# Tongdongq/darwin-gpu

Hardware: AMD Instinct MI355X
Metric: GACT GCUPS (DP cells/s) on ~10 kb PacBio-shape reads (higher is better)
Workload: dtype int16x2 (packed); 1 GPU; ecoli10x_self_overlap; tile_size=320, tile_overlap=120, scoring=+1/-1/-1/-1, reads=4642, bases=48503677, candidates=65766, tiles=2185214, parallelism=candidates dealt round-robin over 1 GPU(s), slots_in_flight=4, passes_in_this_process=127, arch=gfx950:sramecc+:xnack-

## Files before the change

darwin-gpu_amd/csrc/gact_coop.hpp:

```cpp
#pragma once

#include "gact_lin.hpp"

namespace gact {

constexpr int kCoopBanks = 2;
constexpr int kCoopJobs = (kBlockThreads / 64) * 8 * kCoopBanks;
static_assert(kCoopJobs == 64, "a walking wave serves every job of its block, one per lane");
constexpr int kCoopCacheStride = 36;

struct CoopJob {
    uint32_t ws_off;
    int R, Q;
    int k0;
    int v0;
    int band_lim;
    uint32_t where;
    int pad_;
};
struct CoopDone { int ref_steps, query_steps, dv, redo; };

template <class L> constexpr size_t coop_bank_words() { return (size_t)L::G::kMaxFlush * L::kWalkQuads * kWsRow * 4; }
template <class L> __host__ constexpr size_t coop_ws_words(int blocks) { return (size_t)blocks * (kBlockThreads / 64) * kCoopBanks * coop_bank_words<L>(); }

template <class L>
__device__ __forceinline__ void coop_walk_batch(const KParams &kp, const uint32_t *__restrict__ ws_all, const CoopJob *jobs, uint32_t *jstate,
                                                CoopDone *done, const uint32_t *stage_all, uint32_t *cache_all)
{
    constexpr int CW = L::kWalkCols, QN = L::kWalkQuads, ROW = kWsRow;
    constexpr int kSeg = StageGeom<L::kSlotsPerLane, L::kLanes>::kSeg;
    constexpr uint32_t kMagic = (65536u + CW - 1) / CW;
    constexpr uint32_t kM = 3u, kI = 2u, kD = 1u;
    typedef __attribute__((address_space(3))) const uint8_t LdsByte;
    typedef __attribute__((address_space(3))) const uint32_t LdsWord;
    const int lane = threadIdx.x & 63;
    uint32_t *scratch = cache_all + lane * kCoopCacheStride;
    LdsByte *cache = (LdsByte *)scratch;
    LdsWord *stage = (LdsWord *)stage_all;
    const int early = kp.early;
    int v_gap, v_mism, v_match;
    asm volatile("s_nop 1\n\tv_mov_b32 %0, %1" : "=v"(v_gap) : "s"(__builtin_amdgcn_readfirstlane(kp.ext)));
    asm volatile("s_nop 1\n\tv_mov_b32 %0, %1" : "=v"(v_mism) : "s"(__builtin_amdgcn_readfirstlane(kp.mismatch)));
    asm volatile("s_nop 1\n\tv_mov_b32 %0, %1" : "=v"(v_match) : "s"(__builtin_amdgcn_readfirstlane(kp.match)));

    const uint32_t st0 = __hip_atomic_load(&jstate[lane], __ATOMIC_RELAXED, __HIP_MEMORY_SCOPE_WORKGROUP);
    bool active = false;
    if ((st0 & 3u) == 1u) active = atomicCAS(&jstate[lane], st0, st0 + 1u) == st0;
    __builtin_amdgcn_fence(__ATOMIC_ACQUIRE, "workgroup");
    if (!__any(active)) return;
    int p0 = 0, kA = 0, nlim_i = 0, nlim_j = 0, nis = 0, njs = 0, v = 0, v0 = 0, band_lim = -1;
    uint32_t ws_off = 0;
    int rpos0 = 0, qpos0 = 0, dir = 0, seg = 0;
    int l = 0, c = 0, k = 0;
    bool go = false, redo = false;
    if (active) {
        const CoopJob jb = jobs[lane];
        const int R = jb.R, Q = jb.Q;
        ws_off = jb.ws_off; v0 = jb.v0; band_lim = jb.band_lim;
        int l0, c0, k0;
        L::walk_start(R, Q, 0, l0, c0, k0);
        k0 = jb.k0;
        p0 = l0 * CW + c0; kA = k0 - l0;
        nlim_i = -imin(early, R); nlim_j = -imin(early, Q);
        const bool rev = (jb.where >> 16) & 1u;
        seg = (int)(jb.where >> 17);
        dir = rev ? -1 : 1;
        rpos0 = (int)(jb.where & 0xffu) + (rev ? 0 : R - 1);
        qpos0 = (int)((jb.where >> 8) & 0xffu) + (rev ? 0 : Q - 1);
        v = v0;
        l = l0; c = c0; k = k0;
        go = (R >= 1) & (Q >= 1) & (early > 0) & (v != 0);
    }
    uint32_t cur = 0, rcode = 0, qcode = 0;
    TbRegion<CW> rg;
    rg.l0 = 0; rg.fbase[0] = rg.fbase[1] = rg.fbase[2] = 0; rg.qbase0 = 0;
    int off0 = 0, off1 = 0;
    auto fetch = [&](int fl, int fc, int fk) {
        const int off = fl == rg.l0 ? off0 : off1;
        const uint32_t row = ((uint32_t)fk >> 3 << 5) + (uint32_t)off;
        const uint32_t w = *(LdsWord *)(cache + (((uint32_t)fc >> 1 << 2) + row));
        return __builtin_amdgcn_ubfe(w, (((uint32_t)fc & 1u) << 4) + 14u - (((uint32_t)fk & 7u) << 1), 2u);
    };
    auto bases = [&]() {
        const int rp = rpos0 + dir * nis, qp = qpos0 + dir * njs;
        const uint32_t rw = stage[seg + (rp >> 4)], qw = stage[seg + kSeg + (qp >> 4)];
        rcode = __builtin_amdgcn_ubfe(rw, ((uint32_t)rp & 15u) << 1, 2u);
        qcode = __builtin_amdgcn_ubfe(qw, ((uint32_t)qp & 15u) << 1, 2u);
    };
#ifdef GACT_STAMPS
    unsigned long long n_trips = 0, n_lane_trips = 0;
#endif
    while (__any(go)) {
        if (go) {
            tb_refill_oct<CW, QN, ROW>(ws_all, ws_off, scratch, l, c, k, rg);
            off0 = 4 * (-8 * rg.fbase[0] - 4 * rg.qbase0);
            off1 = 4 * (16 - 8 * rg.fbase[1] - 4 * (QN - 2));
            cur = fetch(l, c, k);
            bases();
        }
#pragma unroll 1
        for (int m = 0; m < 8; m++) {
            if (!__any(go)) break;
#ifdef GACT_STAMPS
            n_trips++; n_lane_trips += (unsigned long long)__builtin_popcountll(__ballot(go));
#endif
            if (go) {
                const bool diag = cur == kM;
                const int sub = rcode == qcode ? v_match : v_mism;
                v -= diag ? sub : v_gap;
                nis -= cur != kD;
                njs -= cur != kI;
                const int p = imax(p0 + njs, 0);
                l = (int)(__umul24((uint32_t)p, kMagic) >> 16);
                c = p + __mul24(l, -CW);
                k = imax(kA + l + nis, 0);
                if (m == 7) {
                    redo = redo | ((band_lim >= 0) & ((unsigned)(nis - njs + band_lim) > (unsigned)(2 * band_lim)));
                } else {
                    cur = fetch(l, c, k);
                    bases();
                }
                go = !((diag && v == 0) || nis <= nlim_i || njs <= nlim_j || redo);
            }
        }
    }
    if (active) {
        done[lane].ref_steps = -nis; done[lane].query_steps = -njs; done[lane].dv = v0 - v; done[lane].redo = redo ? 1 : 0;
        __builtin_amdgcn_fence(__ATOMIC_RELEASE, "workgroup");
        __hip_atomic_store(&jstate[lane], st0 + 2u, __ATOMIC_RELAXED, __HIP_MEMORY_SCOPE_WORKGROUP);
    }
#ifdef GACT_STAMPS
    {
        const unsigned long long n_jobs = (unsigned long long)__builtin_popcountll(__ballot(active));
        if (lane == 0) { atomicAdd(&g_coop_counts[0], 1ull); atomicAdd(&g_coop_counts[1], n_trips); atomicAdd(&g_coop_counts[2], n_lane_trips);
                         atomicAdd(&g_coop_counts[3], n_jobs); }
    }
#endif
}

template <class L, bool TWO_SETS = false>
__global__ __launch_bounds__(kBlockThreads, 3) void extend_coop_kernel(
    KParams kp, P16Consts kc, SeqSetDev refs, SeqSetDev qfwd, SeqSetDev qrc,
    int same_file, gact_overlap *__restrict__ out, ChainQueues cq,
    uint32_t *__restrict__ ws_all)
{
    using G = typename L::G;
    constexpr int LANES = L::kLanes;
    static_assert(LANES == kGroup && L::kWalkFmt == 3 && L::kEndAligned, "the split linear-gap layout");
    constexpr int kGroupsOfWave = 64 / LANES;
    constexpr int kGroupsPerBlock = (kBlockThreads / 64) * kGroupsOfWave;
    constexpr int kStageWords = StageGeom<L::kSlotsPerLane, LANES>::kWords;
    constexpr int kSeg = StageGeom<L::kSlotsPerLane, LANES>::kSeg;
    static_assert(((kGroupsPerBlock * kCoopBanks * kStageWords) >> 15) == 0, "stage index fits CoopJob::where");
    constexpr int kRefBytes = (G::kRefBytes + 15) & ~15;
    __shared__ __attribute__((aligned(16))) uint8_t lds[kGroupsPerBlock * kRefBytes];
    __shared__ ChainState chain_lds[kGroupsPerBlock][kCoopBanks][kSlots];
    __shared__ __attribute__((aligned(16))) uint32_t stage_lds[kGroupsPerBlock][kCoopBanks][kStageWords];
    __shared__ __attribute__((aligned(16))) CoopJob jobs[kCoopJobs];
    __shared__ CoopDone done[kCoopJobs];
    __shared__ uint32_t jstate[kCoopJobs];
    __shared__ __attribute__((aligned(16))) uint32_t cache_lds[kCoopJobs * kCoopCacheStride];
    __shared__ int bank_lds[kGroupsPerBlock][kCoopBanks][6];
    __shared__ uint32_t walk_lock;

    uint32_t *const lin_lut = LinLutLds<L::kLutWords>::get();
    for (int n = threadIdx.x; n < kCoopJobs; n += kBlockThreads) jstate[n] = 0;
    if (threadIdx.x == 0) walk_lock = 0;
    lin_lut_fill_for_pass<L>(lin_lut, kc, (int)threadIdx.x);
    __syncthreads();

    const int wave_in_block = threadIdx.x >> 6;
    WaveCtx w;
    {
        const int lane = threadIdx.x & 63;
        w.gl = lane & (LANES - 1);
        w.g = lane / LANES;
        w.slot = (blockIdx.x * (kBlockThreads / 64) + wave_in_block) * kGroupsOfWave + w.g;
        w.n_slots = gridDim.x * (kBlockThreads / 64) * kGroupsOfWave;
    }
    const int group_in_block = wave_in_block * kGroupsOfWave + w.g;
    uint8_t *ref8 = lds + group_in_block * kRefBytes;
    uint8_t *q8 = ref8;
    const uint16_t *ref16_lane = reinterpret_cast<const uint16_t *>(ref8) + (L::kRow0 - 1 - w.gl);
    uint32_t *ws_wave = ws_all + (size_t)(blockIdx.x * (kBlockThreads / 64) + wave_in_block) * (kCoopBanks * coop_bank_words<L>());
    const int job_base = (group_in_block * kSlots + (w.gl & 1)) * kCoopBanks;

    for (int b = 0; b < kCoopBanks; b++)
        if (w.gl < kSlots) { chain_lds[group_in_block][b][w.gl].phase = 2; chain_lds[group_in_block][b][w.gl].cand = -1; }
    if (w.gl == 0) {
        int *bt = &bank_lds[group_in_block][0][0];
        for (int n = 0; n < kCoopBanks * 6; n++) bt[n] = 0;
    }
    wave_sync();
    bool exhausted = false;
    int my_bucket = 0;
    int bucket_first = 0;
    if (cq.leave_longest > 0) {
        int acc = 0;
        while (bucket_first < kBuckets && (acc += cq.bucket_count[bucket_first]) <= cq.leave_longest) bucket_first++;
        if (bucket_first >= kBuckets) bucket_first = 0;
    }
    bool second_set = false;
    constexpr bool one_set = !TWO_SETS;
    int idle_polls = 0;
    int rank_turn = 0, rank_cached = 0;
    int bank = 0;
    __builtin_amdgcn_s_setprio(3);
#ifdef GACT_STAMPS
    unsigned long long stamp_acc[8] = {0, 0, 0, 0, 0, 0, 0, 0};
    const unsigned long long tl_start = __builtin_amdgcn_s_memrealtime();
    const unsigned long long tl_cyc0 = __builtin_amdgcn_s_memtime();
    unsigned long long tl_empty = 0;
#endif

    for (;;) {
        ChainState *st = chain_lds[group_in_block][bank];
        GACT_STAMP(t_w0);
        const int *bk = &bank_lds[group_in_block][bank][0];
        const uint32_t want = (uint32_t)__builtin_amdgcn_readfirstlane(bk[4]);
        if (want != 0) {
            const int sv_R[kSlots] = {bk[0], bk[2]}, sv_Q[kSlots] = {bk[1], bk[3]};
            const bool mine = w.gl < kSlots && ((w.gl & 1) ? sv_R[1] : sv_R[0]) > 0;
            const int my_job = job_base + bank;
            const unsigned long long wd0 = __builtin_amdgcn_s_memrealtime();
            for (;;) {
                const uint32_t s = mine ? __hip_atomic_load(&jstate[my_job], __ATOMIC_RELAXED, __HIP_MEMORY_SCOPE_WORKGROUP) : want;
                if (__all(s == want)) break;
                if (__any(mine && (s & 3u) == 1u)) {
                    uint32_t got = 1;
                    if ((threadIdx.x & 63) == 0) got = atomicCAS(&walk_lock, 0u, 1u);
                    got = (uint32_t)__builtin_amdgcn_readfirstlane((int)got);
                    if (got == 0) {
                        __builtin_amdgcn_fence(__ATOMIC_ACQUIRE, "workgroup");
                        coop_walk_batch<L>(kp, ws_all, jobs, jstate, done, &stage_lds[0][0][0], cache_lds);
                        __builtin_amdgcn_fence(__ATOMIC_RELEASE, "workgroup");
                        if ((threadIdx.x & 63) == 0) __hip_atomic_store(&walk_lock, 0u, __ATOMIC_RELAXED, __HIP_MEMORY_SCOPE_WORKGROUP);
                        continue;
                    }
                }
                __builtin_amdgcn_s_sleep(4);
                if (__builtin_amdgcn_s_memrealtime() - wd0 > 200000000ull) {
                    if ((threadIdx.x & 63) == 0) atomicOr(cq.band_redos, 1 << 30);
                    break;
                }
            }
            __builtin_amdgcn_fence(__ATOMIC_ACQUIRE, "workgroup");
            int ref_steps = 0, query_steps = 0, nst = 0, redo = 0;
            ScoreWalk wk;
            wk.score = 0; wk.pend_gap = 0; wk.open_flag = 0; wk.have_left = 0; wk.left_first_gap = 0;
            if (mine) {
                const CoopDone d = done[my_job];
                wk.load(st[w.gl & 1]);
                wk.score += d.dv;
                ref_steps = d.ref_steps; query_steps = d.query_steps; nst = d.ref_steps + d.query_steps; redo = d.redo;
            }
#pragma unroll
            for (int h = 0; h < kSlots; h++) {
                if (sv_R[h] > 0) {
                    ChainState s = st[h];
                    if (__shfl(redo, h, LANES)) {
                        s.full = 1;
                        if (w.gl == 0) atomicAdd(cq.band_redos, 1);
                    } else {
                        s.full = 0;
                        s.n_tiles++;
                        s.cells += (int64_t)sv_R[h] * sv_Q[h];
                        chain_advance<LANES>(s, false, wk, ref_steps, query_steps, nst, h);
                    }
                    wave_sync();
                    if (w.gl == 0) st[h] = s;
                }
                wave_sync();
            }
            wave_sync();
            if (w.gl == 0) bank_lds[group_in_block][bank][4] = 0;
            wave_sync();
        }
        if (bank == 1 && exhausted) {
            ChainState *st0 = chain_lds[group_in_block][0];
#pragma unroll
            for (int h = 0; h < kSlots; h++) {
                const int ph1 = st[h].phase, f0 = st0[0].phase == 2 ? 0 : st0[1].phase == 2 ? 1 : -1;
                wave_sync();
                if (ph1 != 2 && f0 >= 0 && w.gl == 0) {
                    st0[f0] = st[h];
                    st[h].phase = 2; st[h].cand = -1;
                }
                wave_sync();
            }
        }
        GACT_STAMP(t_a);
        PairTile pt;
        bool have[kSlots];
        int Tend_h[kSlots], tB_h[kSlots];
        int longest = 0;
#pragma unroll
        for (int h = 0; h < kSlots; h++) {
            ChainState s = st[h];
            TilePick pk;
            pk.have = false; pk.R = 0; pk.Q = 0; pk.reverse = false; pk.rp0 = 0; pk.qp0 = 0;
            for (int guard = 0; guard < 3 && !pk.have; guard++) {
                if (s.phase == 2) {
                    if (exhausted) break;
                    int cand = -1;
                    for (;;) {
                        const int *q_count = (TWO_SETS && second_set) ? cq.more_count : cq.bucket_count;
                        int *q_pop = (TWO_SETS && second_set) ? cq.more_pop : cq.bucket_pop;
                        const int *q_live = (TWO_SETS && second_set) ? cq.more_live : cq.live;
                        while (my_bucket < kBuckets) {
                            const int bkt = bucket_first + my_bucket - (bucket_first + my_bucket >= kBuckets ? kBuckets : 0);
                            const int cnt = q_count[bkt];
                            int idx = cnt;
                            if (w.gl == 0 && __hip_atomic_load(&q_pop[bkt], __ATOMIC_RELAXED, __HIP_MEMORY_SCOPE_AGENT) < cnt)
                                idx = atomicAdd(&q_pop[bkt], 1);
                            idx = __shfl(idx, 0, LANES);
                            if (idx < cnt) {
                                cand = q_live[(size_t)bkt * cq.live_stride + idx];
                                break;
                            }
                            my_bucket++;
                        }
                        if (cand >= 0 || second_set || one_set) break;
                        if (__hip_atomic_load(cq.more_flag, __ATOMIC_RELAXED, __HIP_MEMORY_SCOPE_AGENT) == 0) break;
                        __builtin_amdgcn_fence(__ATOMIC_ACQUIRE, "agent");
                        second_set = true;
                        my_bucket = 0;
                    }
                    if (cand < 0) {
                        if (second_set || one_set) {
                            exhausted = true;
#ifdef GACT_STAMPS
                            if (!tl_empty) tl_empty = __builtin_amdgcn_s_memrealtime();
#endif
                        }
                        break;
                    }
                    s = cq.states[cand];
                }
                pk = chain_pick(s, kp, same_file, out, w.gl == 0);
            }
            have[h] = pk.have;
            pt.R[h] = pk.R; pt.Q[h] = pk.Q; pt.reverse[h] = pk.reverse;
            pt.rp0[h] = pk.rp0; pt.qp0[h] = pk.qp0; pt.comp[h] = s.comp; pt.shift[h] = 0;
            pt.full[h] = s.full != 0;
            if (pk.have) longest = imax(longest, chain_remaining(s));
            Tend_h[h] = L::last_step(pk.R, pk.Q);
            tB_h[h] = L::first_pointer_step(pk.R, pk.Q, kp.early);
            wave_sync();
            if (w.gl == 0) st[h] = s;
            wave_sync();
        }
        if (w.gl == 0) {
            int *bw = &bank_lds[group_in_block][bank][0];
            bw[0] = have[0] ? pt.R[0] : 0; bw[1] = pt.Q[0]; bw[2] = have[1] ? pt.R[1] : 0; bw[3] = pt.Q[1];
        }
        const bool any_here = have[0] | have[1];
        if (!__any(any_here)) {
            const bool other_busy = __builtin_amdgcn_readfirstlane(bank_lds[group_in_block][bank ^ 1][4]) != 0;
            if (!other_busy) {
                const ChainState *so = chain_lds[group_in_block][bank ^ 1];
                if (__all(exhausted && st[0].phase == 2 && st[1].phase == 2 && so[0].phase == 2 && so[1].phase == 2)) break;
                if (!second_set && !one_set) {
                    __builtin_amdgcn_s_sleep(127);
                    if (++idle_polls > 512) { second_set = true; exhausted = true; my_bucket = kBuckets; }
                }
            }
            bank ^= 1;
            continue;
        }
        const int T_end = wave_max_groups<LANES>(imax(have[0] ? Tend_h[0] : 0, have[1] ? Tend_h[1] : 0));
        const int reach0 = have[0] ? tB_h[0] + (T_end - Tend_h[0]) : 0x7fffffff;
        const int reach1 = have[1] ? tB_h[1] + (T_end - Tend_h[1]) : 0x7fffffff;
        const int tB = wave_min_groups<LANES>(imin(reach0, reach1));
        pt.col_from = imax(imin(have[0] ? pt.Q[0] : 0x7fff, have[1] ? pt.Q[1] : 0x7fff) - kp.early, 0);
        pt.band = kp.band;
        pt.lut = lin_lut;
        pt.shift[0] = have[0] ? T_end - Tend_h[0] : 0;
        pt.shift[1] = have[1] ? T_end - Tend_h[1] : 0;

        GACT_STAMP(t_b);
        uint32_t qb[L::kSlotsPerLane];
        uint32_t *stage = stage_lds[group_in_block][bank];
        load_pair_packed<L::kSlotsPerLane, LANES, typename L::Cols, false, kLinPadRow>(refs, qfwd, qrc, pt, w.gl, ref8, G::kRefBytes, G::kRow0, q8, G::kTileMax, qb,
                                                                          stage, typename L::Cols{});
        wave_sync();
        GACT_STAMP(t_c);

        const int wave_longest = wave_max_groups<LANES>(longest);
        const int ref_longest = ranked_longest(cq, kp, wave_longest, rank_turn, rank_cached);
        const bool rank_hi = kp.prio_bases[0] == 0 ? 16 * wave_longest > (kp.prio_bases[1] >> 8) * ref_longest
                                                   : wave_longest > kp.prio_bases[1];
        const bool rank_mid = kp.prio_bases[0] == 0 ? 16 * wave_longest > (kp.prio_bases[1] & 255) * ref_longest
                                                    : wave_longest > kp.prio_bases[0];
        if (rank_hi) __builtin_amdgcn_s_setprio(2);
        else if (rank_mid) __builtin_amdgcn_s_setprio(1);
        else __builtin_amdgcn_s_setprio(0);
        uint32_t *wsA = ws_wave + (size_t)bank * coop_bank_words<L>() + (w.g * LANES) * 4;
        uint32_t *wsB = wsA + 64 * 4;
        const uint32_t fin = L::template pass<false>(kc, w.gl, ref16_lane, qb, T_end, tB, wsA, wsB, pt);
        __builtin_amdgcn_s_setprio(3);
        const int v0A = (int)(int16_t)(__shfl(fin, L::fin_lane(pt.Q[0]), LANES) & 0xffffu);
        const int v0B = (int)(int16_t)(__shfl(fin, L::fin_lane(pt.Q[1]), LANES) >> 16);
        GACT_STAMP(t_d);
        asm volatile("s_waitcnt vmcnt(0)" ::: "memory");
        GACT_STAMP(t_e);

        const uint32_t wave_seq = (uint32_t)__builtin_amdgcn_readfirstlane(bank_lds[wave_in_block * kGroupsOfWave][0][5]) + 1u;
        if (w.gl < kSlots) {
            const int h = w.gl;
            if (h ? have[1] : have[0]) {
                const int Rh = h ? pt.R[1] : pt.R[0], Qh = h ? pt.Q[1] : pt.Q[0], sh = h ? pt.shift[1] : pt.shift[0];
                int l0, c0, k0;
                L::walk_start(Rh, Qh, L::tile_tB(tB, sh), l0, c0, k0);
                CoopJob *jb = &jobs[job_base + bank];
                jb->ws_off = (uint32_t)((const char *)(h ? wsB : wsA) - (const char *)ws_all);
                jb->R = Rh; jb->Q = Qh; jb->k0 = k0; jb->v0 = h ? v0B : v0A;
                jb->band_lim = ((kp.band & 0xffff) > 0 && !(h ? pt.full[1] : pt.full[0])) ? (kp.band & 0xffff) - kLinWalkSpan : -1;
                const uint32_t seg_index = (uint32_t)((group_in_block * kCoopBanks + bank) * kStageWords + (2 * h) * kSeg);
                constexpr uint32_t kFrontBits = 16u * StageGeom<L::kSlotsPerLane, LANES>::kFront;
                jb->where = (kFrontBits + (uint32_t)((h ? pt.rp0[1] : pt.rp0[0]) & 15)) |
                            ((kFrontBits + (uint32_t)((h ? pt.qp0[1] : pt.qp0[0]) & 15)) << 8) |
                            ((h ? pt.reverse[1] : pt.reverse[0]) ? 1u << 16 : 0u) | (seg_index << 17);
                __builtin_amdgcn_fence(__ATOMIC_RELEASE, "workgroup");
                __hip_atomic_store(&jstate[job_base + bank], (wave_seq << 2) | 1u, __ATOMIC_RELAXED, __HIP_MEMORY_SCOPE_WORKGROUP);
            }
        }
        wave_sync();
        if (w.gl == 0) bank_lds[group_in_block][bank][4] = (int)((wave_seq << 2) | 3u);
        if ((threadIdx.x & 63) == 0) bank_lds[wave_in_block * kGroupsOfWave][0][5] = (int)wave_seq;
        wave_sync();
        GACT_STAMP(t_f);
        GACT_ACC(0, t_a, t_b); GACT_ACC(1, t_b, t_c); GACT_ACC(2, t_c, t_d); GACT_ACC(3, t_d, t_e);
        GACT_ACC(4, t_w0, t_a); GACT_ACC(5, t_e, t_f);
#ifdef GACT_STAMPS
        stamp_acc[6] += 1; stamp_acc[7] += (unsigned long long)(T_end - tB + 1);
#endif
        bank ^= 1;
    }
#ifdef GACT_STAMPS
    if ((threadIdx.x & 63) == 0) {
        for (int k = 0; k < 8; k++) atomicAdd(&g_stamps[k], stamp_acc[k]);
        const int wv = blockIdx.x * (kBlockThreads / 64) + wave_in_block;
        if (wv < 4096) {
            g_timeline[4 * wv] = tl_start; g_timeline[4 * wv + 1] = tl_empty;
            g_timeline[4 * wv + 2] = __builtin_amdgcn_s_memrealtime(); g_timeline[4 * wv + 3] = stamp_acc[6];
            g_wave_cycles[wv] = __builtin_amdgcn_s_memtime() - tl_cyc0;
        }
    }
#endif
}

}
```

Baseline: 9678 GCUPS.

## Software-pipeline cooperative traceback walk with inline LDS reads and relative positions

```diff
diff --git a/darwin-gpu_amd/csrc/gact_coop.hpp b/darwin-gpu_amd/csrc/gact_coop.hpp
--- a/darwin-gpu_amd/csrc/gact_coop.hpp
+++ b/darwin-gpu_amd/csrc/gact_coop.hpp
@@ -1,6 +1,7 @@
 #pragma once
 
 #include "gact_lin.hpp"
+#include "gact_walk_pos.hpp"
 
 namespace gact {
 
@@ -29,7 +30,6 @@
 {
     constexpr int CW = L::kWalkCols, QN = L::kWalkQuads, ROW = kWsRow;
     constexpr int kSeg = StageGeom<L::kSlotsPerLane, L::kLanes>::kSeg;
-    constexpr uint32_t kMagic = (65536u + CW - 1) / CW;
     constexpr uint32_t kM = 3u, kI = 2u, kD = 1u;
     typedef __attribute__((address_space(3))) const uint8_t LdsByte;
     typedef __attribute__((address_space(3))) const uint32_t LdsWord;
@@ -48,7 +48,7 @@
     if ((st0 & 3u) == 1u) active = atomicCAS(&jstate[lane], st0, st0 + 1u) == st0;
     __builtin_amdgcn_fence(__ATOMIC_ACQUIRE, "workgroup");
     if (!__any(active)) return;
-    int p0 = 0, kA = 0, nlim_i = 0, nlim_j = 0, nis = 0, njs = 0, v = 0, v0 = 0, band_lim = -1;
+    int kA = 0, nlim_i = 0, nlim_j = 0, nis = 0, njs = 0, v0 = 0, band_lim = -1;
     uint32_t ws_off = 0;
     int rpos0 = 0, qpos0 = 0, dir = 0, seg = 0;
     int l = 0, c = 0, k = 0;
@@ -60,32 +60,40 @@
         int l0, c0, k0;
         L::walk_start(R, Q, 0, l0, c0, k0);
         k0 = jb.k0;
-        p0 = l0 * CW + c0; kA = k0 - l0;
+        kA = k0 - l0;
         nlim_i = -imin(early, R); nlim_j = -imin(early, Q);
         const bool rev = (jb.where >> 16) & 1u;
         seg = (int)(jb.where >> 17);
         dir = rev ? -1 : 1;
         rpos0 = (int)(jb.where & 0xffu) + (rev ? 0 : R - 1);
         qpos0 = (int)((jb.where >> 8) & 0xffu) + (rev ? 0 : Q - 1);
-        v = v0;
         l = l0; c = c0; k = k0;
-        go = (R >= 1) & (Q >= 1) & (early > 0) & (v != 0);
+        go = (R >= 1) & (Q >= 1) & (early > 0) & (v0 != 0);
     }
     uint32_t cur = 0, rcode = 0, qcode = 0;
     TbRegion<CW> rg;
     rg.l0 = 0; rg.fbase[0] = rg.fbase[1] = rg.fbase[2] = 0; rg.qbase0 = 0;
-    int off0 = 0, off1 = 0;
-    auto fetch = [&](int fl, int fc, int fk) {
-        const int off = fl == rg.l0 ? off0 : off1;
-        const uint32_t row = ((uint32_t)fk >> 3 << 5) + (uint32_t)off;
-        const uint32_t w = *(LdsWord *)(cache + (((uint32_t)fc >> 1 << 2) + row));
-        return __builtin_amdgcn_ubfe(w, (((uint32_t)fc & 1u) << 4) + 14u - (((uint32_t)fk & 7u) << 1), 2u);
+    int cr = 0, cr_min = 0, k_lane = 0, dv = 0;
+    uint32_t off_a = 0, off_d = 0;
+    const uint32_t cache_a = (uint32_t)(uintptr_t)cache;
+    const uint32_t seg_a = (uint32_t)(uintptr_t)(stage + seg);
+    const int dir2 = 2 * dir, rfix2 = 2 * rpos0 + 8 * (int)seg_a, qfix2 = 2 * qpos0 + 8 * (int)seg_a;
+    uint32_t pw = 0, rw = 0, qw = 0;
+    int rp2 = 0, qp2 = 0;
+    auto issue = [&]() {
+        const uint32_t pa = ((uint32_t)k >> 3 << 5) + (((uint32_t)cr << 1) + off_a) + ((uint32_t)walk_lane_before(cr) & off_d);
+        rp2 = walk_pos2(rfix2, dir2, nis); qp2 = walk_pos2(qfix2, dir2, njs);
+        const uint32_t ra = ((uint32_t)rp2 >> 3) & ~3u, qa = ((uint32_t)qp2 >> 3) & ~3u;
+        asm volatile("ds_read_u16 %0, %3\n\t"
+                     "ds_read_b32 %1, %4\n\t"
+                     "ds_read_b32 %2, %5 offset:%6"
+                     : "=&v"(pw), "=&v"(rw), "=&v"(qw) : "v"(pa), "v"(ra), "v"(qa), "n"(4 * kSeg) : "memory");
     };
-    auto bases = [&]() {
-        const int rp = rpos0 + dir * nis, qp = qpos0 + dir * njs;
-        const uint32_t rw = stage[seg + (rp >> 4)], qw = stage[seg + kSeg + (qp >> 4)];
-        rcode = __builtin_amdgcn_ubfe(rw, ((uint32_t)rp & 15u) << 1, 2u);
-        qcode = __builtin_amdgcn_ubfe(qw, ((uint32_t)qp & 15u) << 1, 2u);
+    auto land = [&]() {
+        asm volatile("s_waitcnt lgkmcnt(0)" : "+v"(pw), "+v"(rw), "+v"(qw) :: "memory");
+        cur = __builtin_amdgcn_ubfe(pw, (uint32_t)(__mul24(k, -2) + 14) & 15u, 2u);
+        rcode = __builtin_amdgcn_ubfe(rw, (uint32_t)rp2, 2u);
+        qcode = __builtin_amdgcn_ubfe(qw, (uint32_t)qp2, 2u);
     };
 #ifdef GACT_STAMPS
     unsigned long long n_trips = 0, n_lane_trips = 0;
@@ -93,39 +101,39 @@
     while (__any(go)) {
         if (go) {
             tb_refill_oct<CW, QN, ROW>(ws_all, ws_off, scratch, l, c, k, rg);
-            off0 = 4 * (-8 * rg.fbase[0] - 4 * rg.qbase0);
-            off1 = 4 * (16 - 8 * rg.fbase[1] - 4 * (QN - 2));
-            cur = fetch(l, c, k);
-            bases();
-        }
-#pragma unroll 1
+            off_a = cache_a + (uint32_t)(4 * (-8 * rg.fbase[0] - 4 * rg.qbase0));
+            off_d = cache_a + (uint32_t)(4 * (16 - 8 * rg.fbase[1] - 4 * (QN - 2)) + 2 * CW) - off_a;
+            walk_trip_begin<CW>(l, c, cr, cr_min);
+            k_lane = kA + l;
+            issue();
+            land();
+        }
+#pragma unroll
         for (int m = 0; m < 8; m++) {
-            if (!__any(go)) break;
-#ifdef GACT_STAMPS
-            n_trips++; n_lane_trips += (unsigned long long)__builtin_popcountll(__ballot(go));
-#endif
-            if (go) {
-                const bool diag = cur == kM;
-                const int sub = rcode == qcode ? v_match : v_mism;
-                v -= diag ? sub : v_gap;
-                nis -= cur != kD;
-                njs -= cur != kI;
-                const int p = imax(p0 + njs, 0);
-                l = (int)(__umul24((uint32_t)p, kMagic) >> 16);
-                c = p + __mul24(l, -CW);
-                k = imax(kA + l + nis, 0);
-                if (m == 7) {
-                    redo = redo | ((band_lim >= 0) & ((unsigned)(nis - njs + band_lim) > (unsigned)(2 * band_lim)));
-                } else {
-                    cur = fetch(l, c, k);
-                    bases();
-                }
-                go = !((diag && v == 0) || nis <= nlim_i || njs <= nlim_j || redo);
-            }
-        }
+#ifdef GACT_STAMPS
+            n_trips += __any(go) ? 1ull : 0ull; n_lane_trips += (unsigned long long)__builtin_popcountll(__ballot(go));
+#endif
+            const bool diag = cur == kM;
+            const int sub = rcode == qcode ? v_match : v_mism;
+            const int cost = diag ? sub : v_gap;
+            dv += go ? cost : 0;
+            nis -= (int)(go & (cur != kD));
+            const int dj = (int)(go & (cur != kI));
+            njs -= dj;
+            walk_col_left(cr, cr_min, dj);
+            k = imax(k_lane + nis + walk_lane_before(cr), 0);
+            if (m == 7) {
+                redo = redo | (go & (band_lim >= 0) & ((unsigned)(nis - njs + band_lim) > (unsigned)(2 * band_lim)));
+            } else {
+                issue();
+            }
+            go = go & !((diag && dv == v0) || nis <= nlim_i || njs <= nlim_j || redo);
+            if (m != 7) land();
+        }
+        walk_trip_end<CW>(rg.l0, cr, l, c);
     }
     if (active) {
-        done[lane].ref_steps = -nis; done[lane].query_steps = -njs; done[lane].dv = v0 - v; done[lane].redo = redo ? 1 : 0;
+        done[lane].ref_steps = -nis; done[lane].query_steps = -njs; done[lane].dv = dv; done[lane].redo = redo ? 1 : 0;
         __builtin_amdgcn_fence(__ATOMIC_RELEASE, "workgroup");
         __hip_atomic_store(&jstate[lane], st0 + 2u, __ATOMIC_RELAXED, __HIP_MEMORY_SCOPE_WORKGROUP);
     }
diff --git a/darwin-gpu_amd/csrc/gact_walk_pos.hpp b/darwin-gpu_amd/csrc/gact_walk_pos.hpp
--- /dev/null
+++ b/darwin-gpu_amd/csrc/gact_walk_pos.hpp
@@ -0,0 +1,47 @@
+#pragma once
+
+#if defined(__HIPCC__) || defined(__CUDACC__)
+#define GACT_WALK_FN __host__ __device__ __forceinline__
+#else
+#define GACT_WALK_FN inline
+#endif
+
+namespace gact {
+
+template <int CW>
+GACT_WALK_FN void walk_trip_begin(int l, int c, int &cr, int &cr_min)
+{
+    cr = c;
+#if defined(__HIP_DEVICE_COMPILE__)
+    cr_min = __mul24(l, -CW);
+#else
+    cr_min = -CW * l;
+#endif
+}
+
+GACT_WALK_FN void walk_col_left(int &cr, int cr_min, int dj)
+{
+    const int next = cr - dj;
+    cr = next > cr_min ? next : cr_min;
+}
+
+GACT_WALK_FN int walk_lane_before(int cr) { return cr >> 31; }
+
+template <int CW>
+GACT_WALK_FN void walk_trip_end(int l0, int cr, int &l, int &c)
+{
+    const int before = walk_lane_before(cr);
+    l = l0 + before;
+    c = cr + (before & CW);
+}
+
+GACT_WALK_FN int walk_pos2(int fix2, int dir2, int n)
+{
+#if defined(__HIP_DEVICE_COMPILE__)
+    return __mul24(n, dir2) + fix2;
+#else
+    return n * dir2 + fix2;
+#endif
+}
+
+}
```

Result: faster. 10060 GCUPS, median of 6 (+3.9%).
